# alibasaran/die-e

Measured on AMD Instinct MI355X. Metric: self-play games/sec, higher is better.
Workload: dtype bf16

## Files before the change

die-e_amd/__init__.py:

```python
import ctypes as C
import os

import numpy as np

_HERE = os.path.dirname(os.path.abspath(__file__))
LIB_PATH = os.environ.get("DIEE_LIB") or os.path.join(_HERE, "libdiee.so")

BG_ACTIONS = 1352
BG_PLANES = 144
NO_MOVE = -2
GAME_TTT, GAME_BACKGAMMON = 0, 1
FLAG_REF_QUIRKS = 1
FLAG_INVARIANT_NN = 2
AGENT_RANDOM, AGENT_MODEL = 0, 1
BAND_BOUNDS = (16, 32, 64, 128, 256, 512, 928, 1024)

OK, ERR_ARG, ERR_HIP, ERR_NO_WEIGHTS, ERR_CAPACITY, ERR_UNSUPPORTED = range(6)

BG_STATE = np.dtype([("pts", "i1", 24), ("bar", "u1", 2), ("off", "u1", 2), ("roll", "u1", 2),
                     ("player", "i1"), ("second", "u1")])
assert BG_STATE.itemsize == 32
TTT_ACTIONS, TTT_PLANES = 9, 27
TTT_STATE = np.dtype([("board", "i1", 9), ("player", "i1"), ("pad", "u1", 22)])
assert TTT_STATE.itemsize == 32

EXPORTS = [
    "diee_create", "diee_destroy", "diee_last_error", "diee_version", "diee_set_option", "diee_get_option", "diee_device_pci_bus_id", "diee_weights_count",
    "diee_random_weights", "diee_load_weights", "diee_nn_forward", "diee_mcts_batch", "diee_self_play",
    "diee_self_play_multi", "diee_self_play_refill", "diee_arena", "diee_set_invariant_nn", "diee_train_pack_conv3x3", "diee_train_pack_conv3x3_multi",
    "diee_train_conv3x3", "diee_train_im2col3x3",
    "diee_train_scratch_floats", "diee_train_bn_relu_fwd", "diee_train_bn_relu_bwd", "diee_train_colsum",
    "diee_train_set_bn_coop", "diee_train_bn_coop_timeouts",
    "diee_train_wgrad_scratch_floats", "diee_train_wgrad3x3",
    "diee_free_fragments", "diee_bg_legal_moves", "diee_bg_encode", "diee_bg_decode", "diee_bg_apply",
    "diee_bg_planes", "diee_det_pow",
    "diee_ttt_valid_moves", "diee_ttt_apply_move", "diee_ttt_check_winner", "diee_ttt_planes",
]
DEV_EXPORTS = ["diee_probe_f32", "diee_probe_dice", "diee_dev_conv_bench", "diee_dev_rules_bench", "diee_dev_wave_selftest",
               "diee_dev_last_dispatch", "diee_dev_dispatch_bands"]


class DieeError(RuntimeError):
    def __init__(self, status, msg):
        super().__init__(f"diee status {status}: {msg}")
        self.status = status


class MctsConfig(C.Structure):
    _fields_ = [("iterations", C.c_uint32), ("c", C.c_float), ("round_limit", C.c_uint32),
                ("dir_alpha", C.c_float), ("dir_eps", C.c_float)]

    @classmethod
    def default(cls, iterations=100):
        return cls(iterations=iterations, c=2.0, round_limit=400, dir_alpha=0.3, dir_eps=0.25)


class Stats(C.Structure):
    _fields_ = ([(n, C.c_uint64) for n in ("games", "plies", "move_steps", "nn_evals", "expansions", "children",
                                           "terminal_hits", "depth_sum", "selections", "illegal_decodes",
                                           "max_children", "fragments")]
                + [("seconds", C.c_double), ("nn_seconds", C.c_double), ("conv_seconds", C.c_double),
                   ("conv_launches", C.c_uint64), ("conv_flops", C.c_double),
# ... 77 lines not shown
    L.diee_train_colsum.argtypes = [vp, vp, C.c_int, vp, vp]; L.diee_train_colsum.restype = C.c_int
    L.diee_train_set_bn_coop.argtypes = [C.c_int]; L.diee_train_set_bn_coop.restype = C.c_int
    L.diee_train_bn_coop_timeouts.argtypes = [C.c_int]; L.diee_train_bn_coop_timeouts.restype = C.c_int
    L.diee_train_wgrad_scratch_floats.argtypes = []; L.diee_train_wgrad_scratch_floats.restype = C.c_size_t
    L.diee_train_wgrad3x3.argtypes = [vp, vp, vp, C.c_int, vp, vp]; L.diee_train_wgrad3x3.restype = C.c_int
    L.diee_free_fragments.argtypes = [vp]; L.diee_free_fragments.restype = None
    L.diee_bg_legal_moves.argtypes = [vp, vp, u32, vp, u32, vp]; L.diee_bg_legal_moves.restype = C.c_int
    L.diee_bg_encode.argtypes = [vp, vp, vp, u32, vp]; L.diee_bg_encode.restype = C.c_int
    L.diee_bg_decode.argtypes = [vp, vp, vp, u32, vp]; L.diee_bg_decode.restype = C.c_int
    L.diee_bg_apply.argtypes = [vp, vp, vp, vp, u32]; L.diee_bg_apply.restype = C.c_int
    L.diee_bg_planes.argtypes = [vp, vp, u32, vp]; L.diee_bg_planes.restype = C.c_int
    L.diee_det_pow.argtypes = [vp, vp, vp, u32, vp]; L.diee_det_pow.restype = C.c_int
    L.diee_ttt_valid_moves.argtypes = [vp, vp]; L.diee_ttt_valid_moves.restype = u32
    L.diee_ttt_apply_move.argtypes = [vp, C.c_uint8]; L.diee_ttt_apply_move.restype = None
    L.diee_ttt_check_winner.argtypes = [vp, C.POINTER(C.c_int)]; L.diee_ttt_check_winner.restype = C.c_int
    L.diee_ttt_planes.argtypes = [vp, vp]; L.diee_ttt_planes.restype = None
    L.diee_probe_f32.argtypes = [vp, vp, vp, u32, vp, vp, vp]; L.diee_probe_f32.restype = C.c_int
    L.diee_probe_dice.argtypes = [vp, u64, vp, u32, vp, vp]; L.diee_probe_dice.restype = C.c_int
    L.diee_dev_conv_bench.argtypes = [vp, C.c_int, C.c_int, C.c_int, vp, vp, vp]; L.diee_dev_conv_bench.restype = C.c_int
    L.diee_dev_rules_bench.argtypes = [vp, vp, C.c_uint32, C.c_int, vp, vp]; L.diee_dev_rules_bench.restype = C.c_int
    L.diee_dev_wave_selftest.argtypes = [vp, C.c_uint32, vp]; L.diee_dev_wave_selftest.restype = C.c_int
    L.diee_dev_last_dispatch.argtypes = [vp, vp, u32, vp]; L.diee_dev_last_dispatch.restype = C.c_int
    L.diee_dev_dispatch_bands.argtypes = [vp, C.c_int, vp, u32, vp]; L.diee_dev_dispatch_bands.restype = C.c_int
    if path is None:
        _lib = L
    return L


def device_pci_bus_id(device=0):
    buf = C.create_string_buffer(64)
    st = load_library().diee_device_pci_bus_id(device, buf, 64)
    if st != OK:
        raise DieeError(st, f"diee_device_pci_bus_id({device})")
    return buf.value.decode()


def same_gpu_as_torch(device):
    import torch
    pr = torch.cuda.get_device_properties(device)
    ours = device_pci_bus_id(device).lower()
    if not hasattr(pr, "pci_bus_id"):
        return True, ours, None
    theirs = f"{getattr(pr, 'pci_domain_id', 0):04x}:{pr.pci_bus_id:02x}:{getattr(pr, 'pci_device_id', 0):02x}.0"
    import re
    m = re.fullmatch(r"([0-9a-f]+):([0-9a-f]+):([0-9a-f]+)\.([0-9a-f]+)", ours)
    if not m:
# ... 126 lines not shown
                                         dv.ctypes.data, pw.ctypes.data))
        return sq, dv, pw

    def probe_dice(self, seed, ctr):
        ctr = np.ascontiguousarray(ctr, dtype=np.uint32); n = len(ctr)
        dice = np.zeros((n, 2), dtype=np.uint8); uni = np.zeros(n, dtype=np.float64)
        self._chk(self._L.diee_probe_dice(self._h, seed, ctr.ctypes.data, n, dice.ctypes.data, uni.ctypes.data))
        return dice, uni

    def load_weights(self, blob):
        blob = np.ascontiguousarray(blob, dtype=np.float32)
        self._chk(self._L.diee_load_weights(self._h, blob.ctypes.data, blob.size))

    def forward_t(self, states):
        s = _states(states); n = len(s)
        pol = np.zeros((n, self.n_actions), dtype=np.float32); val = np.zeros(n, dtype=np.float32)
        self._chk(self._L.diee_nn_forward(self._h, s.ctypes.data, n, pol.ctypes.data, val.ctypes.data))
        return pol, val

    def conv_bench(self, G, variant=0, reps=50):
        a, b, f = C.c_float(0), C.c_float(0), C.c_float(0)
        self._chk(self._L.diee_dev_conv_bench(self._h, G, variant, reps, C.byref(a), C.byref(b), C.byref(f)))
        return a.value, b.value, f.value

    def rules_bench(self, states, reps=20):
        s = _states(states)
        us, k = C.c_float(0), C.c_float(0)
        self._chk(self._L.diee_dev_rules_bench(self._h, s.ctypes.data, len(s), reps, C.byref(us), C.byref(k)))
        return us.value, k.value

    def wave_selftest(self, salt=0):
        bad = C.c_uint32(0)
        self._chk(self._L.diee_dev_wave_selftest(self._h, salt, C.byref(bad)))
        return int(bad.value)

    def set_invariant_nn(self, on=True):
        self._chk(self._L.diee_set_invariant_nn(self._h, 1 if on else 0))

    def alpha_mcts_parallel(self, states, cfg, seed=0, step=0, game_ids=None, rounds=None, ref_quirks=True):
        s = _states(states); n = len(s)
        probs = np.zeros((n, self.n_actions), dtype=np.float32)
        nch = np.zeros(n, dtype=np.uint32); rv = np.zeros(n, dtype=np.float32)
        gi = None if game_ids is None else np.ascontiguousarray(game_ids, dtype=np.uint32)
        rd = None if rounds is None else np.ascontiguousarray(rounds, dtype=np.uint32)
        st = Stats()
        self._chk(self._L.diee_mcts_batch(self._h, s.ctypes.data, n, C.byref(cfg), seed, step,
# ... 124 lines not shown
```

die-e_amd/csrc/diee_api.cpp:

```cpp
#include "../../include/diee.h"
#include "../../include/diee_dev.h"
#include "engine.h"
#include "nn_host.h"
#include "launch.h"
#include "ttt_host.h"

#include <mutex>
#include <cstdarg>
#include <cstdio>
#include <cstring>
#include <cstdlib>
#include <new>

using namespace diee;

#define API_BEGIN(ctx)            \
    if (!(ctx)) return DIEE_ERR_ARG; \
    (ctx)->err[0] = 0;            \
    try {
#define API_END(ctx)                                                        \
    }                                                                       \
    catch (const EngineError& e) {                                          \
        snprintf((ctx)->err, sizeof((ctx)->err), "%s", e.what());           \
        return (diee_status)e.code;                                         \
// ... 238 lines not shown
                       uint32_t* retired_round, int8_t* retired_side, diee_bg_state* initial_states, diee_bg_state* final_states,
                       diee_stats* stats) {
    diee_ctx* c = p1 ? p1 : p2;
    API_BEGIN(c)
    if (!cfg) throw EngineError(DIEE_ERR_ARG, "null pointer");
    Engine* host = bg(c);
    Engine* e1 = p1 ? bg(p1) : nullptr;
    Engine* e2 = p2 ? bg(p2) : nullptr;
    if (e1 && e2 && e1->device != e2->device) throw EngineError(DIEE_ERR_ARG, "the two ctxs of an arena call must be on the same device");
    if ((agent1 == DIEE_AGENT_MODEL && !e1) || (agent2 == DIEE_AGENT_MODEL && !e2)) throw EngineError(DIEE_ERR_ARG, "a Model agent needs its ctx");
    host->arena(e1 ? e1->net : nullptr, agent1, e2 ? e2->net : nullptr, agent2, n_games, cfg, temperature, seed, round_limit, max_rounds, flags,
                res, winner, retired_round, retired_side, initial_states, final_states, stats);
    API_END(c)
}

diee_status diee_dev_conv_bench(diee_ctx* c, int G, int variant, int reps, float* us_mode0, float* us_mode1,
                                float* us_forward) {
    API_BEGIN(c)
    HIPCHK(hipSetDevice(bg(c)->device));
    nn_conv_bench(*bg(c), G, variant, reps, us_mode0, us_mode1, us_forward);
    API_END(c)
}

diee_status diee_dev_last_dispatch(diee_ctx* c, diee_dev_launch* out, uint32_t cap, uint32_t* n) {
    API_BEGIN(c)
    if (!out || !n) throw EngineError(DIEE_ERR_ARG, "null pointer");
    Engine* e = bg(c);
    *n = 0;
    if (!e->net) return DIEE_OK;
    for (const auto& d : e->net->last_dispatch) {
        if (*n >= cap) break;
        diee_dev_launch& o = out[(*n)++];
        o.family = d.family; o.geometry = d.geometry; o.boards = d.boards;
        snprintf(o.kernel, sizeof o.kernel, "%s", nn_kernel_name(d.family, d.geometry));
    }
    API_END(c)
}

diee_status diee_dev_dispatch_bands(diee_ctx* c, int upto_boards, diee_dev_band* out, uint32_t cap, uint32_t* n) {
    API_BEGIN(c)
    if (!out || !n || upto_boards < 1) throw EngineError(DIEE_ERR_ARG, "bad arguments");
    *n = 0;
    for (const auto& b : nn_dispatch_bands(*bg(c), upto_boards)) {
        if (*n >= cap) break;
        diee_dev_band& o = out[(*n)++];
        o.boards_min = b.boards_min; o.boards_max = b.boards_max; o.family = b.family; o.geometry = b.geometry;
// ... 103 lines not shown
```

die-e_amd/csrc/engine.cpp:

```cpp
#include "engine.h"

#include <cctype>
#include <cstdlib>
#include <cstring>
#include <vector>

#include "launch.h"

namespace diee {

void free_net(NetWeights*);
void cluster_baton_register(int device, int delta);
void nn_reset_cluster(Engine& e);
void nn_disable_cluster(Engine& e);
void free_search(SearchBufs*);
void pinned_pool_set_cap_mb(size_t mb);
size_t pinned_pool_cap_mb();

namespace {
struct OptEntry { const char* key; int Options::*i; uint32_t Options::*u; std::string Options::*s; };
const OptEntry kOptions[] = {
    {"tower_table", nullptr, nullptr, &Options::tower_table}, {"tower_cl", nullptr, nullptr, &Options::tower_cl},
    {"tower_pair", &Options::tower_pair, nullptr, nullptr}, {"fused_heads", &Options::fused_heads, nullptr, nullptr},
    {"cluster_heads", &Options::cluster_heads, nullptr, nullptr}, {"cluster_init", &Options::cluster_init, nullptr, nullptr},
    {"compact", &Options::compact, nullptr, nullptr}, {"cl_pack", &Options::cl_pack, nullptr, nullptr},
    {"shared_gpu", &Options::shared_gpu, nullptr, nullptr},
    {"cl_grow", &Options::cl_grow, nullptr, nullptr}, {"expand2", &Options::expand2, nullptr, nullptr},
    {"expand2c", &Options::expand2c, nullptr, nullptr}, {"spec_eval", &Options::spec_eval, nullptr, nullptr},
    {"spec_rollout_steps", nullptr, &Options::spec_rollout_steps, nullptr}, {"spec_max_games", nullptr, &Options::spec_max_games, nullptr},
    {"spec_extra_rows", nullptr, &Options::spec_extra_rows, nullptr}, {"spec_child_rows", nullptr, &Options::spec_child_rows, nullptr},
    {"spec_fused_games", nullptr, &Options::spec_fused_games, nullptr}, {"spec_fused_from", nullptr, &Options::spec_fused_from, nullptr},
    {"spec_rows64_from", nullptr, &Options::spec_rows64_from, nullptr}, {"spec_rows128_from", nullptr, &Options::spec_rows128_from, nullptr},
    {"spec_ring_mb", nullptr, &Options::spec_ring_mb, nullptr},
    {"free_eval", &Options::free_eval, nullptr, nullptr}, {"free_min_games", nullptr, &Options::free_min_games, nullptr},
    {"free_max_games", nullptr, &Options::free_max_games, nullptr}, {"free_rows1024_from", nullptr, &Options::free_rows1024_from, nullptr},
    {"free_rollout_steps", nullptr, &Options::free_rollout_steps, nullptr}, {"free_cand_max", nullptr, &Options::free_cand_max, nullptr},
    {"free_ring", nullptr, &Options::free_ring, nullptr}, {"free_iter_cap", nullptr, &Options::free_iter_cap, nullptr}, {"free_cand_x4", nullptr, &Options::free_cand_x4, nullptr},
    {"free_lag_boost", nullptr, &Options::free_lag_boost, nullptr}, {"free_lag_step", nullptr, &Options::free_lag_step, nullptr}, {"free_lds_nodes", nullptr, &Options::free_lds_nodes, nullptr},
    {"path_cap", nullptr, &Options::path_cap, nullptr}, {"nodes_per_expansion", nullptr, &Options::nodes_per_expansion, nullptr},
    {"deliver_stage_rows", nullptr, &Options::deliver_stage_rows, nullptr}, {"deliver_rows_per_game", nullptr, &Options::deliver_rows_per_game, nullptr},
    {"trace_steps", &Options::trace_steps, nullptr, nullptr}, {"trace_dispatch", &Options::trace_dispatch, nullptr, nullptr},
    {"test_starve_at", &Options::test_starve_at, nullptr, nullptr}, {"test_tail_skip", &Options::test_tail_skip, nullptr, nullptr},
    {"pinned_pool_mb", nullptr, nullptr, nullptr},
};
const char kRefillAreas[] = "refill_record_areas";
const OptEntry* find_option(const std::string& key) {
    for (const auto& e : kOptions) if (key == e.key) return &e;
// ... 213 lines not shown
```

die-e_amd/csrc/engine.h:

```cpp
#pragma once
#include <hip/hip_runtime.h>
#include <stdint.h>

#include <stdexcept>
#include <string>
#include <vector>

#include "../../include/diee.h"

namespace diee {

struct EngineError : public std::runtime_error {
    int code;
    EngineError(int c, const std::string& m) : std::runtime_error(m), code(c) {}
};

#define HIPCHK(expr)                                                                              \
    do {                                                                                          \
        hipError_t e_ = (expr);                                                                   \
        if (e_ != hipSuccess)                                                                     \
            throw ::diee::EngineError(DIEE_ERR_HIP, std::string(#expr) + ": " + hipGetErrorString(e_)); \
    } while (0)

template <class T>
// ... 1 lines not shown
    T* p = nullptr;
    size_t cap = 0;
    DevBuf() = default;
    DevBuf(const DevBuf&) = delete;
    DevBuf& operator=(const DevBuf&) = delete;
    ~DevBuf() { if (p) (void)hipFree(p); }
    void ensure(size_t n) {
        if (n <= cap) return;
        if (p) { (void)hipFree(p); p = nullptr; cap = 0; }
        HIPCHK(hipMalloc((void**)&p, n * sizeof(T)));
        cap = n;
    }
    size_t bytes() const { return cap * sizeof(T); }
};

struct NetWeights;
struct SearchBufs;

struct Options {
    std::string tower_table = "default";
    std::string tower_cl = "default";
    int tower_pair = 1;
    int fused_heads = 1, cluster_heads = 1, cluster_init = 1;
    int compact = 1;
    int cl_pack = 1;
    int shared_gpu = 0;
    int cl_grow = 1, expand2 = 1, expand2c = 1;
    int spec_eval = 1;
    uint32_t spec_rollout_steps = 24;
    uint32_t spec_fused_from = 129;
    uint32_t spec_fused_games = 256;
    uint32_t spec_child_rows = 16;
    uint32_t spec_extra_rows = 2;
    uint32_t spec_max_games = 96;
    uint32_t spec_rows64_from = 5, spec_rows128_from = 10;
    int free_eval = 1;
    uint32_t free_min_games = 17, free_max_games = 800;
    uint32_t free_rows1024_from = 200;
    uint32_t free_rollout_steps = 24, free_cand_max = 12;
    uint32_t free_cand_x4 = 8;
    uint32_t free_lag_boost = 4, free_lag_step = 4;
    uint32_t free_iter_cap = 4;
    uint32_t free_ring = 128;
    uint32_t free_lds_nodes = 3072;
    uint32_t spec_ring_mb = 8192;
    uint32_t path_cap = 64, nodes_per_expansion = 128;
// ... 70 lines not shown
```

die-e_amd/csrc/launch.h:

```cpp
#pragma once
#include <hip/hip_runtime.h>
#include <stdint.h>

#include "search_types.h"

namespace diee {

void launch_legal_moves(hipStream_t st, const void* states, uint32_t n, uint32_t* plays, uint32_t cap,
                        uint32_t* counts, uint32_t* overflow);
void launch_encode(hipStream_t st, const void* states, const uint32_t* plays, uint32_t n, uint32_t* codes);
void launch_decode(hipStream_t st, const void* states, const uint32_t* codes, uint32_t n, uint32_t* plays);
void launch_apply(hipStream_t st, void* states, const uint32_t* plays, const uint8_t* dice, uint32_t n);
void launch_planes(hipStream_t st, const void* states, uint32_t n, float* out);
void launch_wave_selftest(hipStream_t st, uint32_t* mismatches, uint32_t salt);
void launch_probe_f32(hipStream_t st, const float* a, const float* b, uint32_t n, float* sq, float* dv, float* pw);
void launch_probe_dice(hipStream_t st, uint64_t seed, const uint32_t* ctr, uint32_t n, uint8_t* dice, double* uni);

struct GrowReq { Tree T; Slots S; Segs G; uint32_t n, it; };

void nn_setup_kernels();
void nn_set_conv_variant(int v);
void launch_planes_bf16(hipStream_t st, const void* states, uint32_t n, uint16_t* out);
void launch_conv3x3(hipStream_t st, int c_in, int mode, const uint16_t* act, const void* wpack, const float* bias,
                    const uint16_t* res, uint16_t* out, float* out_v, int G, int N);
// ... 8 lines not shown
constexpr int kClusterMaxGroups = 64;
bool launch_tower_cluster(hipStream_t st, int device, int boards_per_group, uint16_t* X, uint16_t* H, const void* wt, const float* bias,
                          int G, uint32_t* sync, uint32_t* err, const void* states, const void* winit, const float* binit,
                          const void* whead = nullptr, const float* bhead = nullptr, const void* wfc = nullptr, const float* bfc = nullptr,
                          float* hv = nullptr, float* logits = nullptr, const GrowReq* grow = nullptr, bool* grown = nullptr, bool pack = true,
                          const uint32_t* n_rows_dev = nullptr, uint32_t* rows_log = nullptr);
int train_stripes(int M);
void launch_bn_relu_fwd(hipStream_t st, const uint16_t* x, const uint16_t* res, const float* gamma, const float* beta, float* partial,
                        float* save_mean, float* save_invstd, float* run_mean, float* run_var, float momentum, float eps,
                        uint16_t* y, int M);
void launch_bn_relu_bwd(hipStream_t st, const uint16_t* dy, const uint16_t* y, const uint16_t* x, const float* gamma,
                        const float* mean, const float* invstd, float* partial, float* dgamma, float* dbeta, uint16_t* dx,
                        uint16_t* dres, float* dx_colsum , int M);
void bn_coop_set(int on);
int bn_coop_get();
int bn_coop_poll_timeouts(int clear);
size_t wgrad_scratch_floats();
void launch_wgrad3x3(hipStream_t st, const uint16_t* x, const uint16_t* dy, float* partial, float* dw, int boards);
void launch_colsum(hipStream_t st, const uint16_t* a, float* partial, float* out, int M);
void launch_pack_conv_w(hipStream_t st, const float* w_oihw, uint16_t* wpack, int transpose);
constexpr int kMaxPackLayers = 64;
void launch_pack_conv_w_multi(hipStream_t st, const float* const* w, int n, uint16_t* wpack);
void launch_im2col3x3(hipStream_t st, const uint16_t* x, uint16_t* col, int boards);
void launch_policy_fc(hipStream_t st, const uint16_t* hp, const void* wpack, const float* bias, float* logits, int G,
                      const uint32_t* n_rows = nullptr);
void launch_tower_compact(hipStream_t st, const void* wt16, const float* bias, int n_upper, const void* states,
                          const void* winit16, const float* binit, const void* whead16, const float* bhead, uint16_t* hp, float* hv,
                          const uint32_t* row_slot, const uint32_t* n_rows, uint16_t* pair_ex = nullptr, uint32_t* err = nullptr);
void launch_tower_free(hipStream_t st, const void* wt16, const float* bias, int n_upper, const void* states, const void* winit16, const float* binit,
                       const void* whead16, const float* bhead, uint16_t* hp, float* hv, const uint32_t* row_idx, const uint32_t* n_rows,
                       uint16_t* pair_ex = nullptr, uint32_t* err = nullptr);
void launch_tower_pair_counted(hipStream_t st, const void* wt16, const float* bias, int G, const void* states, const void* winit16, const float* binit,
                               const void* whead16, const float* bhead, uint16_t* hp, float* hv, uint16_t* ex, uint32_t* err, const uint32_t* n_rows);
bool launch_tower_pair(hipStream_t st, int boards_per_pair , const void* wt16, const float* bias, int G, const void* states, const void* winit16,
                       const float* binit, const void* whead16, const float* bhead, uint16_t* hp, float* hv, uint16_t* ex, uint32_t* err);
bool tower_pair_device_ok(int device);
size_t tower_pair_exchange_bytes();
int tower_pair_max_boards(int boards_per_pair);
void launch_softmax_value(hipStream_t st, const float* logits, const float* hv, const float* wv, float* policy,
                          float* value, int G);

void launch_init_roots(hipStream_t st, const Tree& T, const Slots& S, uint32_t n);
struct ExpandVariant { bool two = true, two_c = true; };
void launch_expand(hipStream_t st, const Tree& T, const Slots& S, const Segs& G, uint32_t n, uint32_t it, const SearchParams& P,
                   uint32_t next_it, float c, bool pre_grown = false, ExpandVariant v = ExpandVariant{});
void launch_tail(hipStream_t st, const Tree& T, const Slots& S, const Segs& G, uint32_t n, const SearchParams& P, float c, const Tail& L, uint32_t q);
void launch_free(hipStream_t st, const Tree& T, const Slots& S, const Segs& G, uint32_t n, const SearchParams& P, float c, const Free& F, uint32_t q);
uint32_t free_lds_nodes_for(uint32_t n, uint32_t cus);
// ... 22 lines not shown
```

die-e_amd/csrc/nn_conv_kernels.hip:

```cpp
#include "nn_common.h"

namespace diee {

__global__ void k_planes_bf16(const BgState* __restrict__ states, uint32_t n, uint16_t* __restrict__ out) {
    const uint32_t i = blockIdx.x * blockDim.x + threadIdx.x;
    if (i >= n * 24u) return;
    const BgState s = states[i / 24u];
    const int p = (int)(i % 24u);
    uint32_t w[8];
#pragma unroll
    for (int c = 0; c < 8; ++c) {
        const uint32_t lo = 2 * c < 6 ? f2bf(bg_plane_dev(s, 2 * c, p)) : 0u;
        const uint32_t hi = 2 * c + 1 < 6 ? f2bf(bg_plane_dev(s, 2 * c + 1, p)) : 0u;
        w[c] = lo | (hi << 16);
    }
    u32x4* o = (u32x4*)(out + (size_t)i * 16);
    o[0] = u32x4{w[0], w[1], w[2], w[3]};
    o[1] = u32x4{w[4], w[5], w[6], w[7]};
}

template <int C_IN, int MODE, int GT, int NW>
__global__ __launch_bounds__(64 * NW) void k_conv3x3(const uint16_t* __restrict__ act,
                                                     const u32x4* __restrict__ wpack,
                                                     const float* __restrict__ bias,
// ... 257 lines not shown
            o[j] = (uint32_t)f2bf(x0) | ((uint32_t)f2bf(x1) << 16);
            v[2 * j] = x0; v[2 * j + 1] = x1;
        }
        if (MODE == 2) {
            const int g = gr / 24, p = gr % 24;
            if (nslice == 0) *(u32x4*)(out + (size_t)g * 768 + p * 32 + c8 * 8) = o;
            else if (c8 == 0) { float* ov = out_v + (size_t)g * 72 + p * 3; ov[0] = v[0]; ov[1] = v[1]; ov[2] = v[2]; }
        } else {
            *(u32x4*)(out + (size_t)gr * N + nslice * 32 + c8 * 8) = o;
        }
    }
}

__global__ __launch_bounds__(64) void k_policy_fc(const uint16_t* __restrict__ hp,
                                                  const u32x4* __restrict__ wpack,
                                                  const float* __restrict__ bias,
                                                  float* __restrict__ logits,
                                                  int G, const uint32_t* __restrict__ n_rows ) {
    const int g0 = blockIdx.x * 32;
    if (n_rows) { G = (int)*n_rows; if (g0 >= G) return; }
    policy_fc_tile(hp, (const fc_u32x4*)wpack, bias, logits, G, g0, blockIdx.y, threadIdx.x);
}

__global__ __launch_bounds__(64) void k_softmax_value(const float* __restrict__ logits, const float* __restrict__ hv,
                                                      const float* __restrict__ wv ,
                                                      float* __restrict__ policy, float* __restrict__ value, int G) {
    const int g = blockIdx.x, lane = threadIdx.x;
    if (g >= G) return;
    const float* lr = logits + (size_t)g * 1352;
    float M, inv;
    softmax_consts(lr, lane, M, inv);
    for (int a = lane; a < 1352; a += 64) policy[(size_t)g * 1352 + a] = softmax_prob(lr[a], M, inv);
    const float v = value_head(hv + (size_t)g * 72, wv, lane);
    if (lane == 0) value[g] = v;
}

template <int C_IN, int GT, int NC>
static constexpr int conv_lds_bytes() {
    constexpr int rows = GT * 24;
    constexpr int a = (rows + 1) * (C_IN * 2 + 16) + 16 * 34 + 128;
    constexpr int o = rows * (NC * 4 + 16);
    return a > o ? a : o;
}

template <int C_IN, int MODE, int GT, int NW>
static void conv_launch(hipStream_t st, const uint16_t* act, const void* wpack, const float* bias, const uint16_t* res,
// ... 125 lines not shown
}
__global__ void k_im2col3x3(const uint16_t* __restrict__ x, uint16_t* __restrict__ col, int M) {
    const size_t i = (size_t)blockIdx.x * blockDim.x + threadIdx.x;
    if (i >= (size_t)M * 9 * 32) return;
    const int ch = (int)(i & 31), t = (int)((i >> 5) % 9), row = (int)(i / (9 * 32));
    const int p = row % 24, y = p / 6, xx = p % 6, dy = t / 3 - 1, dx = t % 3 - 1;
    u32x4 v = {0u, 0u, 0u, 0u};
    if ((unsigned)(y + dy) < 4u && (unsigned)(xx + dx) < 6u) v = *(const u32x4*)(x + (size_t)(row + 6 * dy + dx) * 256 + ch * 8);
    *(u32x4*)(col + (size_t)row * 2304 + t * 256 + ch * 8) = v;
}
void launch_pack_conv_w(hipStream_t st, const float* w, uint16_t* out, int transpose) {
    hipLaunchKernelGGL(k_pack_conv_w, dim3(8 * 144 * 64 * 8 / 256), dim3(256), 0, st, w, out, transpose);
}
void launch_pack_conv_w_multi(hipStream_t st, const float* const* w, int n, uint16_t* out) {
    PackPtrs p{};
    for (int i = 0; i < n; ++i) p.w[i] = w[i];
    hipLaunchKernelGGL(k_pack_conv_w_multi, dim3(128, 2, n), dim3(256), 0, st, p, out);
}
void launch_im2col3x3(hipStream_t st, const uint16_t* x, uint16_t* col, int boards) {
    const size_t n = (size_t)boards * 24 * 9 * 32;
    hipLaunchKernelGGL(k_im2col3x3, dim3((unsigned)((n + 255) / 256)), dim3(256), 0, st, x, col, boards * 24);
}

void launch_policy_fc(hipStream_t st, const uint16_t* hp, const void* wpack, const float* bias, float* logits, int G,
                      const uint32_t* n_rows) {
    if (G <= 0) return;
    hipLaunchKernelGGL(k_policy_fc, dim3((G + 31) / 32, 43), dim3(64), 0, st, hp, (const u32x4*)wpack, bias, logits, G, n_rows);
}

void launch_softmax_value(hipStream_t st, const float* logits, const float* hv, const float* wv, float* policy,
                          float* value, int G) {
    if (G <= 0) return;
    hipLaunchKernelGGL(k_softmax_value, dim3(G), dim3(64), 0, st, logits, hv, wv, policy, value, G);
}

}
```

die-e_amd/csrc/nn_host.cpp:

```cpp
#include <algorithm>
#include <cmath>
#include <cstdio>
#include <cstdlib>
#include <cstring>
#include <mutex>

#include "bg_device.h"
#include "engine.h"
#include "launch.h"
#include "nn_host.h"

namespace diee {

namespace {

constexpr int F = 256, BLOCKS = 19, A = 1352, CIN = 6, PH = 32, VH = 3;
constexpr int kFullRestBoards = 928;

struct ConvOff { size_t w, b; int cout, cin; };
struct BnOff { size_t g, b, m, v; int c; };
struct BlobLayout {
    ConvOff init_conv; BnOff init_bn;
    ConvOff c1[BLOCKS], c2[BLOCKS]; BnOff b1[BLOCKS], b2[BLOCKS];
    ConvOff p_conv; BnOff p_bn; size_t p_fcw, p_fcb;
// ... 103 lines not shown
    { const float bd = 1.0f / std::sqrt((float)(VH * 24)); uni(L.v_fcw, VH * 24, -bd, bd); uni(L.v_fcb, 1, -bd, bd); }
}

void free_net(NetWeights* n) { delete n; }

template <class Row>
static void parse_table(const std::string& t, std::vector<Row>& out) {
    out.clear();
    size_t pos = 0;
    while (pos < t.size() && t != "none") {
        const size_t c = t.find(':', pos), e2 = t.find(',', pos);
        if (c == std::string::npos) break;
        out.push_back({atoi(t.substr(pos, c - pos).c_str()), atoi(t.substr(c + 1, (e2 == std::string::npos ? t.size() : e2) - c - 1).c_str())});
        if (e2 == std::string::npos) break;
        pos = e2 + 1;
    }
}

void Engine::apply_options() {
    if (!net) return;
    NetWeights& W = *net;
    W.fused_heads = opt.fused_heads != 0; W.cluster_heads = opt.cluster_heads != 0; W.cluster_init = opt.cluster_init != 0;
    W.compact = opt.compact != 0; W.cl_pack = opt.cl_pack != 0; W.trace_dispatch = opt.trace_dispatch != 0;
    const bool handoffs = !opt.shared_gpu && !W.starved;
    bool pair = opt.tower_pair != 0 && handoffs;
    if (pair && !tower_pair_device_ok(device)) {
        pair = false;
        if (!W.told_no_pair) fprintf(stderr, "[diee] pair tower: device %d is not 8 XCDs x 32 CUs (a partition?); using the single-workgroup geometries\n", device);
        W.told_no_pair = true;
    }
    W.pair_tower = pair;
    if (opt.tower_table == "default") W.tower_table = pair ? NetWeights::default_tower_table() : NetWeights::default_tower_table_no_pair();
    else {
        std::vector<NetWeights::TowerRule> t;
        parse_table(opt.tower_table, t);
        for (const auto& r : t)
            if (r.geometry != 10 && r.geometry != 11 && !tower_geometry_supported(r.geometry)) {
                opt.tower_table = "default";
                throw EngineError(DIEE_ERR_ARG, "option tower_table: geometry " + std::to_string(r.geometry) + " is not in this build (product: 3, 5, 6, 14 and "
                                  "10 / 11 = the pair tower; python die-e_amd/build.py --dev has the others)");
            }
        W.tower_table = t;
    }
    if (!pair) for (auto& r : W.tower_table) if (r.geometry == 10 || r.geometry == 11) r.geometry = 3;
    if (!handoffs) W.cluster_table.clear();
    else if (opt.tower_cl == "default") W.cluster_table = NetWeights::default_cluster_table();
// ... 214 lines not shown
            kind = 2;
        } else {
            kind = 0;
            W.last_dispatch.push_back({0, 0, G});
            for (int i = 0; i < BLOCKS; ++i) {
                launch_conv3x3(st, 256, 0, actX, W.wl(1 + 2 * i), W.bl(1 + 2 * i), nullptr, actH, nullptr, G, 256);
                launch_conv3x3(st, 256, 1, actH, W.wl(2 + 2 * i), W.bl(2 + 2 * i), actX, actX, nullptr, G, 256);
            }
        }
    }
    if (trace_dispatch)
        fprintf(stderr, "[diee] forward of boards %d..%d: %s (fused geometry %d, conv variant table entries %zu / %zu)\n", off, off + G,
                kind == 1 ? "fused tower" : kind == 2 ? "cluster tower" : "per-layer kernels", tgeom, W.tower_table.size(), W.cluster_table.size());
    if (sample) {
        HIPCHK(hipEventRecord(ev1, st));
        W.pending.push_back({ev0, ev1, 38.0 * 2.0 * G * 24.0 * 2304.0 * 256.0, kind == 0 ? 38 : 1, (kind == 1 && tower_geometry_is_full_chip(tgeom)) ? 3 : kind, -1, G});
    }
    if (!heads_done) launch_conv3x3(st, 256, 2, actX, W.wconv[39].p, W.bconv[39].p, nullptr, hp, hv, G, 64);
    return fc_done;
}

static void fc_launch(Engine& e, const uint16_t* hp, float* logits, int G, const uint32_t* n_rows = nullptr) {
    NetWeights& W = *e.net;
    launch_policy_fc(e.stream, hp, W.wfc.p, W.bfc.p, logits, G, n_rows);
}

bool nn_forward(Engine& e, const void* states_dev, int G, float* policy_dev, float* value_dev, const NnRows* rows) {
    if (!e.net || !e.net->loaded) throw EngineError(DIEE_ERR_NO_WEIGHTS, "diee_load_weights has not been called");
    if (G <= 0) return false;
    NetWeights& W = *e.net;
    nn_reserve(e, G);
    W.last_dispatch.clear();
    hipStream_t st = e.stream;
    const int tg = W.tower_geometry_for(G);
    const bool one_full_pass = G > kFullRestBoards && G <= W.full_chip_boards;
    if (rows && W.compact && !policy_dev && G > W.compact_above && !one_full_pass && tg >= 2 && W.cluster_init && W.fused_heads) {
        const uint32_t seq = (uint32_t)(W.forward_count & (kRowsLog - 1));
        const bool sample = W.sample_every > 0 && (W.forward_count++ % W.sample_every) == 0;
        W.rows_log.ensure(kRowsLog);
        launch_row_map(st, rows->skip, (uint32_t)G, rows->row_slot, rows->slot_row, rows->n_rows, W.rows_log.p, seq);
        hipEvent_t ev0 = nullptr, ev1 = nullptr;
        if (sample) { ev0 = W.get_event(); ev1 = W.get_event(); HIPCHK(hipEventRecord(ev0, st)); }
        uint16_t* pex = pair_exchange(e);
        if (pex) W.cluster_used = true;
        launch_tower_compact(st, W.wtower16.p, W.btower.p, G, states_dev, W.winit16.p, W.bconv[0].p, W.whead16.p, W.bconv[39].p,
                             W.hp.p, W.hv.p, rows->row_slot, rows->n_rows, pex, e.flags_dev.p);
        W.last_dispatch.push_back({1, -1, G});
// ... 207 lines not shown
            while (b < (int)DIEE_BANDS - 1 && p.boards > bounds[b]) ++b;
            W.band_seconds[b] += ms * 1e-3; W.band_launches[b] += 1; W.band_flops[b] += p.flops; W.band_flops_demanded[b] += flops_dem;
        }
        W.free_events.push_back(p.a); W.free_events.push_back(p.b);
    }
    W.pending.clear();
    if (stats) {
        stats->conv_seconds = W.conv_seconds; stats->conv_launches = W.conv_launches; stats->conv_flops = W.conv_flops;
        stats->tower_seconds = W.tower_seconds; stats->tower_launches = W.tower_launches; stats->tower_flops = W.tower_flops;
        stats->cluster_seconds = W.cluster_seconds; stats->cluster_launches = W.cluster_launches; stats->cluster_flops = W.cluster_flops;
        stats->full_seconds = W.full_seconds; stats->full_launches = W.full_launches; stats->full_flops = W.full_flops;
        for (int b = 0; b < (int)DIEE_BANDS; ++b) { stats->band_seconds[b] = W.band_seconds[b]; stats->band_launches[b] = W.band_launches[b]; stats->band_flops[b] = W.band_flops[b]; stats->band_flops_demanded[b] = W.band_flops_demanded[b]; }
    }
}
void nn_reset_timing(Engine& e) {
    if (!e.net) return;
    e.net->conv_seconds = 0; e.net->conv_launches = 0; e.net->conv_flops = 0; e.net->forward_count = 0;
    e.net->tower_seconds = 0; e.net->tower_launches = 0; e.net->tower_flops = 0;
    e.net->cluster_seconds = 0; e.net->cluster_launches = 0; e.net->cluster_flops = 0;
    e.net->full_seconds = 0; e.net->full_launches = 0; e.net->full_flops = 0;
    for (int b = 0; b < (int)DIEE_BANDS; ++b) { e.net->band_seconds[b] = 0; e.net->band_launches[b] = 0; e.net->band_flops[b] = 0; e.net->band_flops_demanded[b] = 0; }
}

#ifdef DIEE_DEV_BUILD
void nn_conv_bench(Engine& e, int G, int variant, int reps, float* us_mode0, float* us_mode1, float* us_forward) {
    if (!e.net || !e.net->loaded) throw EngineError(DIEE_ERR_NO_WEIGHTS, "diee_load_weights has not been called");
    NetWeights& W = *e.net;
    nn_reserve(e, G);
    hipStream_t st = e.stream;
    const size_t M = (size_t)((G + 7) / 8 * 8) * 24;
    const int fill = getenv("DIEE_BENCH_ZERO") ? 0 : 0x3c;
    HIPCHK(hipMemsetAsync(W.actX.p, fill, M * 256 * 2, st));
    HIPCHK(hipMemsetAsync(W.actH.p, fill, M * 256 * 2, st));
    hipEvent_t a, b;
    HIPCHK(hipEventCreate(&a)); HIPCHK(hipEventCreate(&b));
    nn_set_conv_variant(variant);
    float ms = 0.f;
    for (int mode = 0; mode < 2; ++mode) {
        for (int r = -3; r < reps; ++r) {
            if (r == 0) HIPCHK(hipEventRecord(a, st));
            const int layer = 1 + ((r + 3) % 38);
            launch_conv3x3(st, 256, mode, mode ? W.actH.p : W.actX.p, W.wl(layer), W.bl(layer),
                           mode ? W.actX.p : nullptr, mode ? W.actX.p : W.actH.p, nullptr, G, 256);
        }
        HIPCHK(hipEventRecord(b, st));
        HIPCHK(hipEventSynchronize(b));
// ... 77 lines not shown
```

die-e_amd/csrc/nn_host.h:

```cpp
#pragma once
#include <vector>

#include "engine.h"

namespace diee {

struct GrowReq;

struct NetWeights {
    DevBuf<uint16_t> wconv[40];
    DevBuf<float> bconv[40];
    DevBuf<uint16_t> wtower;
    DevBuf<uint16_t> wtower16;
    DevBuf<float> btower;
    DevBuf<uint16_t> winit16, whead16;
    uint16_t* wl(int layer) { return (layer >= 1 && layer <= 38) ? wtower.p + (size_t)(layer - 1) * 8 * 144 * 64 * 8 : wconv[layer].p; }
    float* bl(int layer) { return (layer >= 1 && layer <= 38) ? btower.p + (size_t)(layer - 1) * 256 : bconv[layer].p; }
    struct TowerRule { int min_games, geometry; };
    static std::vector<TowerRule> default_tower_table() { return {{928, 5}, {640, 14}, {512, 6}, {256, 10}, {40, 11}}; }
    static std::vector<TowerRule> default_tower_table_no_pair() { return {{928, 5}, {640, 14}, {416, 6}, {256, 3}}; }
    std::vector<TowerRule> tower_table = default_tower_table();
    DevBuf<uint16_t> pair_ex;
    bool pair_tower = true;
    bool starved = false;
    bool told_no_pair = false;
    struct Launched { int family, geometry, boards; };
    std::vector<Launched> last_dispatch;
    bool cl_pack = true;
    bool trace_dispatch = false;
    bool invariant = false;
    int tower_geometry_for(int G) const {
        for (const auto& r : tower_table) if (G > r.min_games) return r.geometry;
        return invariant ? 3 : -1;
    }
    struct ClusterRule { int max_games, boards_per_group; };
    static std::vector<ClusterRule> default_cluster_table() { return {{32, 1}, {64, 2}, {128, 4}, {256, 8}}; }
    std::vector<ClusterRule> cluster_table = default_cluster_table();
    DevBuf<uint32_t> cl_sync;
    bool cluster_used = false;
    int full_chip_boards = 1024;
    bool fused_heads = true;
    bool cluster_init = true;
    const struct GrowReq* grow_req = nullptr;
    bool grow_done = false;
    bool cluster_heads = true;
    DevBuf<uint16_t> wfc;
    DevBuf<float> bfc, wv;
    bool loaded = false;
    DevBuf<uint16_t> x16, actX, actH, hp;
    DevBuf<float> hv, logits;
    int cap_games = 0;
    struct Pending { hipEvent_t a, b; double flops; int launches; int kind; int rows_seq; int boards; int dem_seq = -1; int step = -1; };
    bool compact = true;
    int compact_above = 256;
    DevBuf<uint32_t> rows_log;
    int cur_step = -1;
    DevBuf<uint32_t> dem_log;
    std::vector<Pending> pending;
    std::vector<hipEvent_t> free_events;
    int sample_every = 17;
    uint64_t forward_count = 0;
    double conv_seconds = 0, conv_flops = 0, tower_seconds = 0, tower_flops = 0, cluster_seconds = 0, cluster_flops = 0;
    uint64_t conv_launches = 0, tower_launches = 0, cluster_launches = 0;
    double full_seconds = 0, full_flops = 0;
    uint64_t full_launches = 0;
    double band_flops_demanded[DIEE_BANDS] = {};
    double band_seconds[DIEE_BANDS] = {}, band_flops[DIEE_BANDS] = {};
    uint64_t band_launches[DIEE_BANDS] = {};
    hipEvent_t get_event() {
// ... 7 lines not shown
};

constexpr uint32_t kRowsLog = 1u << 20;
struct NnRows { const uint8_t* skip; uint32_t* row_slot; uint32_t* slot_row; uint32_t* n_rows; };
void nn_reserve(Engine& e, int G);
bool nn_forward(Engine& e, const void* states_dev, int G, float* policy_dev, float* value_dev, const NnRows* rows = nullptr);
struct NetHeads { const float* logits; const float* hv; const float* wv; };
NetHeads nn_heads(Engine& e, int G);
const char* nn_kernel_name(int family, int geometry);
struct DispatchBand { int boards_min, boards_max, family, geometry; };
std::vector<DispatchBand> nn_dispatch_bands(Engine& e, int upto);
bool nn_tail_available(Engine& e, int G_upper, int n);
bool nn_forward_tail(Engine& e, const void* states_dev, int G_upper, const uint32_t* n_rows_dev, float* hv_out, float* logits_out, int boards_band,
                     const uint32_t* n_dem_dev = nullptr);
bool nn_free_available(Engine& e, int n);
void nn_forward_free(Engine& e, const void* arena_states, const uint32_t* rows_idx, const uint32_t* n_rows_dev, int rows_upper, float* hv_out, float* logits_out, int boards_band,
                     const uint32_t* n_dem_dev = nullptr);
bool nn_cluster_used(Engine& e);
void nn_disable_cluster(Engine& e);
void nn_reset_cluster(Engine& e);
void nn_harvest(Engine& e, diee_stats* stats, const std::vector<unsigned long long>* step_log = nullptr);
void nn_reset_timing(Engine& e);
void nn_conv_bench(Engine& e, int G, int variant, int reps, float* us_mode0, float* us_mode1, float* us_forward);

}
```

include/diee_dev.h:

```cpp
#ifndef DIEE_DEV_H
#define DIEE_DEV_H
#include "diee.h"
#ifdef __cplusplus
extern "C" {
#endif

diee_status diee_probe_f32(diee_ctx*, const float* a, const float* b, uint32_t n,
                           float* sqrt_a, float* a_div_b, float* pow_ab);
diee_status diee_probe_dice(diee_ctx*, uint64_t seed, const uint32_t* ctr , uint32_t n,
                            uint8_t* dice , double* uniform );

diee_status diee_dev_conv_bench(diee_ctx*, int G, int variant, int reps, float* us_mode0,
                                float* us_mode1, float* us_forward);
diee_status diee_dev_rules_bench(diee_ctx*, const diee_bg_state* states, uint32_t n, int reps,
                                 float* us_legal_moves, float* mean_plays);

typedef struct { int family, geometry, boards; char kernel[120]; } diee_dev_launch;
typedef struct { int boards_min, boards_max, family, geometry; char kernel[120]; } diee_dev_band;
diee_status diee_dev_last_dispatch(diee_ctx*, diee_dev_launch* out, uint32_t cap, uint32_t* n);
diee_status diee_dev_dispatch_bands(diee_ctx*, int upto_boards, diee_dev_band* out, uint32_t cap, uint32_t* n);

diee_status diee_dev_wave_selftest(diee_ctx*, uint32_t salt, uint32_t* mismatches);

#ifdef __cplusplus
}
#endif
#endif
```

Before: 124.9.

## Add LDS-staged multi-wave policy FC kernel and make it the default

Adds a policy fully-connected kernel where each workgroup of 2 or 4 waves loads a shared 32-row activation tile into LDS once (with XOR swizzling) and each wave then computes one 32-column output slice with MFMA, prefetching weights into registers. This replaces the old one-wave-per-slice kernel, in which every wave re-read the activation rows from global memory. The default option policy_fc=1 picks 2 or 4 waves by batch size. It also adds bench, run and ablation entry points, at the cost of 48KB of LDS per block, which may reduce occupancy.

Result: no change. 125.4 (median of 6 runs) (+0.3%).

```diff
diff --git a/die-e_amd/__init__.py b/die-e_amd/__init__.py
--- a/die-e_amd/__init__.py
+++ b/die-e_amd/__init__.py
@@ -37,7 +37,7 @@
     "diee_ttt_valid_moves", "diee_ttt_apply_move", "diee_ttt_check_winner", "diee_ttt_planes",
 ]
 DEV_EXPORTS = ["diee_probe_f32", "diee_probe_dice", "diee_dev_conv_bench", "diee_dev_rules_bench", "diee_dev_wave_selftest",
-               "diee_dev_last_dispatch", "diee_dev_dispatch_bands"]
+               "diee_dev_last_dispatch", "diee_dev_dispatch_bands", "diee_dev_fc_bench", "diee_dev_fc_run", "diee_dev_last_fc"]
 
 
 class DieeError(RuntimeError):
@@ -161,6 +161,9 @@
     L.diee_dev_wave_selftest.argtypes = [vp, C.c_uint32, vp]; L.diee_dev_wave_selftest.restype = C.c_int
     L.diee_dev_last_dispatch.argtypes = [vp, vp, u32, vp]; L.diee_dev_last_dispatch.restype = C.c_int
     L.diee_dev_dispatch_bands.argtypes = [vp, C.c_int, vp, u32, vp]; L.diee_dev_dispatch_bands.restype = C.c_int
+    L.diee_dev_fc_bench.argtypes = [vp, C.c_int, C.c_int, C.c_int, vp]; L.diee_dev_fc_bench.restype = C.c_int
+    L.diee_dev_fc_run.argtypes = [vp, vp, C.c_int, C.c_int, C.c_int, vp]; L.diee_dev_fc_run.restype = C.c_int
+    L.diee_dev_last_fc.argtypes = [vp, vp, vp]; L.diee_dev_last_fc.restype = C.c_int
     if path is None:
         _lib = L
     return L
@@ -333,6 +336,22 @@
         a, b, f = C.c_float(0), C.c_float(0), C.c_float(0)
         self._chk(self._L.diee_dev_conv_bench(self._h, G, variant, reps, C.byref(a), C.byref(b), C.byref(f)))
         return a.value, b.value, f.value
+
+    def fc_bench(self, rows, variant=1, reps=200):
+        us = C.c_float(0)
+        self._chk(self._L.diee_dev_fc_bench(self._h, rows, variant, reps, C.byref(us)))
+        return us.value
+
+    def fc_run(self, hp, logits, n_rows=-1, variant=1):
+        hp = np.ascontiguousarray(hp, dtype=np.uint16)
+        assert hp.ndim == 2 and hp.shape[1] == 768 and logits.dtype == np.float32 and logits.shape == (len(hp), 1352) and logits.flags.c_contiguous
+        self._chk(self._L.diee_dev_fc_run(self._h, hp.ctypes.data, len(hp), n_rows, variant, logits.ctypes.data))
+        return logits
+
+    def last_fc(self):
+        v, r = C.c_int(-1), C.c_int(0)
+        self._chk(self._L.diee_dev_last_fc(self._h, C.byref(v), C.byref(r)))
+        return v.value, r.value
 
     def rules_bench(self, states, reps=20):
         s = _states(states)
diff --git a/die-e_amd/csrc/diee_api.cpp b/die-e_amd/csrc/diee_api.cpp
--- a/die-e_amd/csrc/diee_api.cpp
+++ b/die-e_amd/csrc/diee_api.cpp
@@ -284,6 +284,29 @@
     API_END(c)
 }
 
+diee_status diee_dev_fc_bench(diee_ctx* c, int rows, int variant, int reps, float* us) {
+    API_BEGIN(c)
+    HIPCHK(hipSetDevice(bg(c)->device));
+    nn_fc_bench(*bg(c), rows, variant, reps, us);
+    API_END(c)
+}
+
+diee_status diee_dev_fc_run(diee_ctx* c, const uint16_t* hp, int rows, int n_rows, int variant, float* logits) {
+    API_BEGIN(c)
+    HIPCHK(hipSetDevice(bg(c)->device));
+    nn_fc_run(*bg(c), hp, rows, n_rows, variant, logits);
+    API_END(c)
+}
+
+diee_status diee_dev_last_fc(diee_ctx* c, int* variant, int* rows) {
+    API_BEGIN(c)
+    if (!variant || !rows) throw EngineError(DIEE_ERR_ARG, "null pointer");
+    Engine* e = bg(c);
+    *variant = e->net ? e->net->last_fc.variant : -1;
+    *rows = e->net ? e->net->last_fc.rows : 0;
+    API_END(c)
+}
+
 diee_status diee_dev_last_dispatch(diee_ctx* c, diee_dev_launch* out, uint32_t cap, uint32_t* n) {
     API_BEGIN(c)
     if (!out || !n) throw EngineError(DIEE_ERR_ARG, "null pointer");
diff --git a/die-e_amd/csrc/engine.cpp b/die-e_amd/csrc/engine.cpp
--- a/die-e_amd/csrc/engine.cpp
+++ b/die-e_amd/csrc/engine.cpp
@@ -23,6 +23,7 @@
     {"tower_table", nullptr, nullptr, &Options::tower_table}, {"tower_cl", nullptr, nullptr, &Options::tower_cl},
     {"tower_pair", &Options::tower_pair, nullptr, nullptr}, {"fused_heads", &Options::fused_heads, nullptr, nullptr},
     {"cluster_heads", &Options::cluster_heads, nullptr, nullptr}, {"cluster_init", &Options::cluster_init, nullptr, nullptr},
+    {"policy_fc", &Options::policy_fc, nullptr, nullptr},
     {"compact", &Options::compact, nullptr, nullptr}, {"cl_pack", &Options::cl_pack, nullptr, nullptr},
     {"shared_gpu", &Options::shared_gpu, nullptr, nullptr},
     {"cl_grow", &Options::cl_grow, nullptr, nullptr}, {"expand2", &Options::expand2, nullptr, nullptr},
diff --git a/die-e_amd/csrc/engine.h b/die-e_amd/csrc/engine.h
--- a/die-e_amd/csrc/engine.h
+++ b/die-e_amd/csrc/engine.h
@@ -47,6 +47,7 @@
     std::string tower_cl = "default";
     int tower_pair = 1;
     int fused_heads = 1, cluster_heads = 1, cluster_init = 1;
+    int policy_fc = 1;
     int compact = 1;
     int cl_pack = 1;
     int shared_gpu = 0;
diff --git a/die-e_amd/csrc/launch.h b/die-e_amd/csrc/launch.h
--- a/die-e_amd/csrc/launch.h
+++ b/die-e_amd/csrc/launch.h
@@ -54,8 +54,8 @@
 constexpr int kMaxPackLayers = 64;
 void launch_pack_conv_w_multi(hipStream_t st, const float* const* w, int n, uint16_t* wpack);
 void launch_im2col3x3(hipStream_t st, const uint16_t* x, uint16_t* col, int boards);
-void launch_policy_fc(hipStream_t st, const uint16_t* hp, const void* wpack, const float* bias, float* logits, int G,
-                      const uint32_t* n_rows = nullptr);
+bool launch_policy_fc(hipStream_t st, const uint16_t* hp, const void* wpack, const float* bias, float* logits, int G,
+                      const uint32_t* n_rows = nullptr, int variant = 1);
 void launch_tower_compact(hipStream_t st, const void* wt16, const float* bias, int n_upper, const void* states,
                           const void* winit16, const float* binit, const void* whead16, const float* bhead, uint16_t* hp, float* hv,
                           const uint32_t* row_slot, const uint32_t* n_rows, uint16_t* pair_ex = nullptr, uint32_t* err = nullptr);
diff --git a/die-e_amd/csrc/nn_conv_kernels.hip b/die-e_amd/csrc/nn_conv_kernels.hip
--- a/die-e_amd/csrc/nn_conv_kernels.hip
+++ b/die-e_amd/csrc/nn_conv_kernels.hip
@@ -303,6 +303,114 @@
     policy_fc_tile(hp, (const fc_u32x4*)wpack, bias, logits, G, g0, blockIdx.y, threadIdx.x);
 }
 
+template <int W>
+__global__ __launch_bounds__(64 * W) void k_policy_fc_lds(const uint16_t* __restrict__ hp,
+                                                          const u32x4* __restrict__ wpack,
+                                                          const float* __restrict__ bias,
+                                                          float* __restrict__ logits,
+                                                          int G, const uint32_t* __restrict__ n_rows ) {
+    extern __shared__ __attribute__((aligned(16))) char smem[];
+    constexpr int NA = 48 / W, RG = 8 / W;
+    const int g0 = blockIdx.x * 32;
+    if (n_rows) G = (int)*n_rows;
+    if (g0 >= G) return;
+    const int tid = threadIdx.x, lane = tid & 63, wave = __builtin_amdgcn_readfirstlane(tid >> 6);
+    const int s = blockIdx.y * W + wave;
+    const bool live = s < 43;
+    const fc_u32x4* wp = (const fc_u32x4*)wpack + (size_t)(live ? s : 0) * 48 * 64 + lane;
+    const int pc = lane & 15, kl = pc >> 1;
+    const char* arow[RG];
+    int adst[RG];
+#pragma unroll
+    for (int k = 0; k < RG; ++k) {
+        const int r = 4 * (wave * RG + k) + (lane >> 4);
+        const int row = g0 + r < G ? g0 + r : G - 1;
+        arow[k] = (const char*)hp + (size_t)row * 1536 + pc * 16;
+        adst[k] = kl * 1024 + ((((pc & 1) << 5) | r) ^ kl) * 16;
+    }
+    const int ard = lane * 16;
+    constexpr int PF = 24, AD = 6;
+    fc_u32x4 av[NA], bq[PF];
+#pragma unroll
+    for (int i = 0; i < NA; ++i) av[i] = *(const fc_u32x4*)(arow[i % RG] + (i / RG) * 256);
+    __builtin_amdgcn_sched_barrier(0);
+    if (live) {
+#pragma unroll
+        for (int i = 0; i < PF; ++i) bq[i] = wp[i * 64];
+    }
+    __builtin_amdgcn_sched_barrier(0);
+#pragma unroll
+    for (int i = 0; i < NA; ++i) {
+        const int m8 = i / RG;
+        *(fc_u32x4*)(smem + (adst[i % RG] ^ ((m8 & 1) << 7)) + m8 * 8192) = av[i];
+    }
+    __syncthreads();
+    if (!live) return;
+    fc_f32x16 acc;
+#pragma unroll
+    for (int i = 0; i < 16; ++i) acc[i] = 0.0f;
+    fc_bf16x8 a[AD];
+#pragma unroll
+    for (int i = 0; i < AD; ++i) a[i] = *(const fc_bf16x8*)(smem + (ard ^ ((i & 15) << 4)) + i * 1024);
+#pragma unroll
+    for (int ks = 0; ks < 48; ++ks) {
+        __builtin_amdgcn_sched_barrier(0);
+        acc = __builtin_amdgcn_mfma_f32_32x32x16_bf16(a[ks % AD], __builtin_bit_cast(fc_bf16x8, bq[ks % PF]), acc, 0, 0, 0);
+        if (ks + AD < 48) a[ks % AD] = *(const fc_bf16x8*)(smem + (ard ^ (((ks + AD) & 15) << 4)) + (ks + AD) * 1024);
+        if (ks + PF < 48) bq[ks % PF] = wp[(ks + PF) * 64];
+    }
+    __builtin_amdgcn_sched_barrier(0);
+    const int n = s * 32 + (lane & 31);
+    if (n >= 1352) return;
+    const float bv = bias[n];
+#pragma unroll
+    for (int i = 0; i < 16; ++i) {
+        const int g = g0 + (i & 3) + 8 * (i >> 2) + 4 * (lane >> 5);
+        if (g < G) logits[(size_t)g * 1352 + n] = acc[i] + bv;
+    }
+}
+
+#ifdef DIEE_DEV_BUILD
+template <int ABL>
+__global__ __launch_bounds__(64) void k_policy_fc_ablate(const uint16_t* __restrict__ hp, const u32x4* __restrict__ wpack, const float* __restrict__ bias,
+                                                         float* __restrict__ logits, int G) {
+    const int g0 = blockIdx.x * 32, nslice = blockIdx.y, lane = threadIdx.x;
+    int row = g0 + (lane & 31);
+    if (row >= G) row = G - 1;
+    const int base = g0 + 32 <= G ? g0 : G - 32;
+    const uint16_t* ap = ABL == 1 ? hp + (size_t)base * 768 + lane * 8 : hp + (size_t)row * 768 + (lane >> 5) * 8;
+    const fc_u32x4* wp = (const fc_u32x4*)wpack + (size_t)nslice * 48 * 64 + lane;
+    fc_f32x16 acc;
+#pragma unroll
+    for (int i = 0; i < 16; ++i) acc[i] = 0.0f;
+    uint32_t mix = 0;
+#pragma unroll
+    for (int half = 0; half < 2; ++half) {
+        fc_u32x4 avq[24], bvq[24];
+#pragma unroll
+        for (int i = 0; i < 24; ++i) {
+            avq[i] = *(const fc_u32x4*)(ap + (half * 24 + i) * (ABL == 1 ? 512 : 16));
+            if (ABL == 2) bvq[i] = fc_u32x4{(uint32_t)lane, 0x3c3c3c3cu, (uint32_t)i, 0x3c3c3c3cu};
+            else bvq[i] = wp[(half * 24 + i) * 64];
+        }
+        __builtin_amdgcn_sched_barrier(0);
+#pragma unroll
+        for (int i = 0; i < 24; ++i) {
+            if (ABL == 3) mix ^= avq[i].x ^ avq[i].y ^ avq[i].z ^ avq[i].w ^ bvq[i].x ^ bvq[i].y ^ bvq[i].z ^ bvq[i].w;
+            else acc = __builtin_amdgcn_mfma_f32_32x32x16_bf16(__builtin_bit_cast(fc_bf16x8, avq[i]), __builtin_bit_cast(fc_bf16x8, bvq[i]), acc, 0, 0, 0);
+        }
+    }
+    const int n = nslice * 32 + (lane & 31);
+    if (n >= 1352) return;
+    const float bv = bias[n] + (ABL == 3 ? (float)(mix & 1) : 0.0f);
+#pragma unroll
+    for (int i = 0; i < 16; ++i) {
+        const int g = g0 + (i & 3) + 8 * (i >> 2) + 4 * (lane >> 5);
+        if (g < G) logits[(size_t)g * 1352 + n] = acc[i] + bv;
+    }
+}
+#endif
+
 __global__ __launch_bounds__(64) void k_softmax_value(const float* __restrict__ logits, const float* __restrict__ hv,
                                                       const float* __restrict__ wv ,
                                                       float* __restrict__ policy, float* __restrict__ value, int G) {
@@ -474,10 +582,35 @@
     hipLaunchKernelGGL(k_im2col3x3, dim3((unsigned)((n + 255) / 256)), dim3(256), 0, st, x, col, boards * 24);
 }
 
-void launch_policy_fc(hipStream_t st, const uint16_t* hp, const void* wpack, const float* bias, float* logits, int G,
-                      const uint32_t* n_rows) {
-    if (G <= 0) return;
-    hipLaunchKernelGGL(k_policy_fc, dim3((G + 31) / 32, 43), dim3(64), 0, st, hp, (const u32x4*)wpack, bias, logits, G, n_rows);
+static int fc_lds_waves_for(int G) { return G <= 256 ? 2 : 4; }
+
+template <int W>
+static void fc_lds_launch(hipStream_t st, const uint16_t* hp, const void* wpack, const float* bias, float* logits, int G, const uint32_t* n_rows) {
+    hipLaunchKernelGGL(k_policy_fc_lds<W>, dim3((G + 31) / 32, (43 + W - 1) / W), dim3(64 * W), 48 * 1024, st, hp, (const u32x4*)wpack, bias, logits,
+                       G, n_rows);
+}
+
+bool launch_policy_fc(hipStream_t st, const uint16_t* hp, const void* wpack, const float* bias, float* logits, int G,
+                      const uint32_t* n_rows, int variant) {
+    if (G <= 0) return true;
+    if (variant == 0) {
+        hipLaunchKernelGGL(k_policy_fc, dim3((G + 31) / 32, 43), dim3(64), 0, st, hp, (const u32x4*)wpack, bias, logits, G, n_rows);
+        return true;
+    }
+#ifdef DIEE_DEV_BUILD
+    if (variant >= 10 && variant <= 12 && G >= 32 && !n_rows) {
+        const dim3 grid((G + 31) / 32, 43);
+        if (variant == 10) hipLaunchKernelGGL(k_policy_fc_ablate<1>, grid, dim3(64), 0, st, hp, (const u32x4*)wpack, bias, logits, G);
+        else if (variant == 11) hipLaunchKernelGGL(k_policy_fc_ablate<2>, grid, dim3(64), 0, st, hp, (const u32x4*)wpack, bias, logits, G);
+        else hipLaunchKernelGGL(k_policy_fc_ablate<3>, grid, dim3(64), 0, st, hp, (const u32x4*)wpack, bias, logits, G);
+        return true;
+    }
+#endif
+    const int waves = variant == 1 ? fc_lds_waves_for(G) : variant - 100;
+    if (waves == 2) fc_lds_launch<2>(st, hp, wpack, bias, logits, G, n_rows);
+    else if (waves == 4) fc_lds_launch<4>(st, hp, wpack, bias, logits, G, n_rows);
+    else return false;
+    return true;
 }
 
 void launch_softmax_value(hipStream_t st, const float* logits, const float* hv, const float* wv, float* policy,
diff --git a/die-e_amd/csrc/nn_host.cpp b/die-e_amd/csrc/nn_host.cpp
--- a/die-e_amd/csrc/nn_host.cpp
+++ b/die-e_amd/csrc/nn_host.cpp
@@ -149,6 +149,7 @@
     NetWeights& W = *net;
     W.fused_heads = opt.fused_heads != 0; W.cluster_heads = opt.cluster_heads != 0; W.cluster_init = opt.cluster_init != 0;
     W.compact = opt.compact != 0; W.cl_pack = opt.cl_pack != 0; W.trace_dispatch = opt.trace_dispatch != 0;
+    W.policy_fc = opt.policy_fc != 0 ? 1 : 0;
     const bool handoffs = !opt.shared_gpu && !W.starved;
     bool pair = opt.tower_pair != 0 && handoffs;
     if (pair && !tower_pair_device_ok(device)) {
@@ -409,7 +410,9 @@
 
 static void fc_launch(Engine& e, const uint16_t* hp, float* logits, int G, const uint32_t* n_rows = nullptr) {
     NetWeights& W = *e.net;
-    launch_policy_fc(e.stream, hp, W.wfc.p, W.bfc.p, logits, G, n_rows);
+    W.last_fc = {W.policy_fc, G};
+    if (!launch_policy_fc(e.stream, hp, W.wfc.p, W.bfc.p, logits, G, n_rows, W.policy_fc))
+        throw EngineError(DIEE_ERR_ARG, "option policy_fc = " + std::to_string(W.policy_fc) + ": no such policy FC kernel");
 }
 
 bool nn_forward(Engine& e, const void* states_dev, int G, float* policy_dev, float* value_dev, const NnRows* rows) {
@@ -663,6 +666,48 @@
     for (int b = 0; b < (int)DIEE_BANDS; ++b) { e.net->band_seconds[b] = 0; e.net->band_launches[b] = 0; e.net->band_flops[b] = 0; e.net->band_flops_demanded[b] = 0; }
 }
 
+void nn_fc_bench(Engine& e, int rows, int variant, int reps, float* us) {
+    if (!e.net || !e.net->loaded) throw EngineError(DIEE_ERR_NO_WEIGHTS, "diee_load_weights has not been called");
+    if (rows <= 0 || reps <= 0 || !us) throw EngineError(DIEE_ERR_ARG, "bad arguments");
+    NetWeights& W = *e.net;
+    nn_reserve(e, rows);
+    hipStream_t st = e.stream;
+    HIPCHK(hipMemsetAsync(W.hp.p, 0x3c, (size_t)rows * 768 * 2, st));
+    hipEvent_t a, b;
+    HIPCHK(hipEventCreate(&a)); HIPCHK(hipEventCreate(&b));
+    bool ok = true;
+    for (int r = -3; r < reps && ok; ++r) {
+        if (r == 0) HIPCHK(hipEventRecord(a, st));
+        ok = launch_policy_fc(st, W.hp.p, W.wfc.p, W.bfc.p, W.logits.p, rows, nullptr, variant);
+    }
+    float ms = 0.f;
+    if (ok) {
+        HIPCHK(hipEventRecord(b, st));
+        HIPCHK(hipEventSynchronize(b));
+        HIPCHK(hipEventElapsedTime(&ms, a, b));
+    }
+    (void)hipEventDestroy(a); (void)hipEventDestroy(b);
+    if (!ok) throw EngineError(DIEE_ERR_UNSUPPORTED, "diee_dev_fc_bench: variant " + std::to_string(variant) + " is not in this build");
+    HIPCHK(hipGetLastError());
+    *us = ms * 1e3f / reps;
+}
+void nn_fc_run(Engine& e, const uint16_t* hp, int rows, int n_rows, int variant, float* logits) {
+    if (!e.net || !e.net->loaded) throw EngineError(DIEE_ERR_NO_WEIGHTS, "diee_load_weights has not been called");
+    if (rows <= 0 || n_rows > rows || !hp || !logits || (variant != 0 && variant != 1 && variant < 100)) throw EngineError(DIEE_ERR_ARG, "bad arguments");
+    NetWeights& W = *e.net;
+    nn_reserve(e, rows);
+    e.tmp_d.ensure(sizeof(uint32_t));
+    const uint32_t count = n_rows >= 0 ? (uint32_t)n_rows : 0u;
+    e.h2d(W.hp.p, hp, (size_t)rows * 768);
+    e.h2d(W.logits.p, logits, (size_t)rows * 1352);
+    e.h2d((uint32_t*)e.tmp_d.p, &count, 1);
+    const bool ok = launch_policy_fc(e.stream, W.hp.p, W.wfc.p, W.bfc.p, W.logits.p, rows, n_rows >= 0 ? (const uint32_t*)e.tmp_d.p : nullptr, variant);
+    if (!ok) throw EngineError(DIEE_ERR_UNSUPPORTED, "diee_dev_fc_run: variant " + std::to_string(variant) + " is not in this build");
+    HIPCHK(hipGetLastError());
+    e.d2h(logits, W.logits.p, (size_t)rows * 1352);
+    e.sync();
+}
+
 #ifdef DIEE_DEV_BUILD
 void nn_conv_bench(Engine& e, int G, int variant, int reps, float* us_mode0, float* us_mode1, float* us_forward) {
     if (!e.net || !e.net->loaded) throw EngineError(DIEE_ERR_NO_WEIGHTS, "diee_load_weights has not been called");
diff --git a/die-e_amd/csrc/nn_host.h b/die-e_amd/csrc/nn_host.h
--- a/die-e_amd/csrc/nn_host.h
+++ b/die-e_amd/csrc/nn_host.h
@@ -45,6 +45,8 @@
     bool grow_done = false;
     bool cluster_heads = true;
     DevBuf<uint16_t> wfc;
+    int policy_fc = 1;
+    struct LaunchedFc { int variant = -1, rows = 0; } last_fc;
     DevBuf<float> bfc, wv;
     bool loaded = false;
     DevBuf<uint16_t> x16, actX, actH, hp;
@@ -98,5 +100,7 @@
 void nn_harvest(Engine& e, diee_stats* stats, const std::vector<unsigned long long>* step_log = nullptr);
 void nn_reset_timing(Engine& e);
 void nn_conv_bench(Engine& e, int G, int variant, int reps, float* us_mode0, float* us_mode1, float* us_forward);
+void nn_fc_bench(Engine& e, int rows, int variant, int reps, float* us);
+void nn_fc_run(Engine& e, const uint16_t* hp, int rows, int n_rows, int variant, float* logits);
 
 }
diff --git a/include/diee_dev.h b/include/diee_dev.h
--- a/include/diee_dev.h
+++ b/include/diee_dev.h
@@ -12,6 +12,9 @@
 
 diee_status diee_dev_conv_bench(diee_ctx*, int G, int variant, int reps, float* us_mode0,
                                 float* us_mode1, float* us_forward);
+diee_status diee_dev_fc_bench(diee_ctx*, int rows, int variant, int reps, float* us);
+diee_status diee_dev_fc_run(diee_ctx*, const uint16_t* hp, int rows, int n_rows, int variant, float* logits);
+diee_status diee_dev_last_fc(diee_ctx*, int* variant, int* rows);
 diee_status diee_dev_rules_bench(diee_ctx*, const diee_bg_state* states, uint32_t n, int reps,
                                  float* us_legal_moves, float* mean_plays);
 
```
